# DLR-RM/AugmentedAutoencoder

Measured on AMD Instinct MI355X. Metric: crops/sec (encode+codebook-NN), 128x128x3 vs 92232x128 codebook, 1/8 GPU, higher is better.
Workload: dtype f32; 1 GPU; configs[1]: single object per GPU, batch=256 uint8 128x128x3 crops, HIP 4-conv encoder -> 128-d + cosine-NN vs 92232x128 fp32 codebook, top-1; batch_per_gpu=256, codebook_rows=92232, latent=128, parallelism=single GPU

## Files before the change

augmentedautoencoder_amd/csrc/kernels/conv_winograd_f32.h:

```cpp
#pragma once
#include <type_traits>

#include "multi_launch.h"

namespace aae {

struct ConvWinoArgs {
    const float* x;
    const float* U;
    const float* bias;
    const float* bn_scale;
    const float* bn_shift;
    float* out;
    int B, H, W, Cin, Cout, Ho, Wo;
    int eh, ew;
    int mode;
    int relu;
    int blocks_x, blocks_y;
    int regions;
    int xcd_cols;
#ifdef AAE_WINO_STAMPS
    long long* stamps;
#endif
};
#ifdef AAE_WINO_STAMPS
constexpr int kWinoStampSlots = 48;
#define AAE_WINO_STAMP(a, slot) do { if ((threadIdx.x & 63) == 0) (a).stamps[((size_t)blockIdx.x * 8 + (threadIdx.x >> 6)) * aae::kWinoStampSlots + (slot)] = aae::clock_ticks(); } while (0)
#else
#define AAE_WINO_STAMP(a, slot) do {} while (0)
#endif
inline unsigned wino_grid_blocks(int regions, int nbn, int xcd_cols) {
    if (xcd_cols <= 0) return (unsigned)regions * (unsigned)nbn;
    const int region_groups = 8 / (nbn / xcd_cols);
    return 8u * (unsigned)xcd_cols * (unsigned)((regions + region_groups - 1) / region_groups);
}
inline bool wino_xcd_cols_valid(int nbn, int xcd_cols) {
    return xcd_cols >= 1 && nbn % xcd_cols == 0 && (nbn / xcd_cols) <= 8 && 8 % (nbn / xcd_cols) == 0;
}

template <int GEOM>
struct WinoGeom;
template <>
struct WinoGeom<0> {
    static constexpr int kImages = 1, kRows = 18, kCols = 18, kRowPitch = 12, kParityPitch = 220, kImagePitch = 2 * 220;
};
template <>
struct WinoGeom<1> {
    static constexpr int kImages = 4, kRows = 10, kCols = 10, kRowPitch = 6, kParityPitch = 60, kImagePitch = 128;
};
template <int GEOM>
constexpr int wino_plane_units() { return WinoGeom<GEOM>::kImages * WinoGeom<GEOM>::kImagePitch + 1; }
template <int GEOM>
constexpr int wino_stage_units() { return 8 * wino_plane_units<GEOM>(); }
template <int GEOM>
constexpr int wino_smem_bytes() { return 2 * wino_stage_units<GEOM>() * 16; }

struct ConvWinoLayerArgs {
    ConvWinoArgs c;
    const float* U4[4];
};
struct ConvWinoObject {
    const float* x;
    float* out;
    const float* U4[4];
    const float* bias;
    const float* bn_scale;
    const float* bn_shift;
    int B, pad_;
};
struct ConvWinoMultiArgs {
    ConvWinoArgs c;
    MultiRange range;
    ConvWinoObject obj[kMultiMax];
};
template <int GEOM>
constexpr int wino_layer_stage_bytes() { return 2 * 4 * wino_plane_units<GEOM>() * 16; }
template <int GEOM>
constexpr int wino_layer_smem_bytes() { return wino_layer_stage_bytes<GEOM>() + 4 * 64 * 64 * 4; }


#ifndef AAE_WINO_DECLARATIONS_ONLY

#if defined(__HIP_DEVICE_COMPILE__)
__device__ __forceinline__ f32x2 wino_pk_add(f32x2 a, f32x2 b) {
    f32x2 r;
    asm("v_pk_add_f32 %0, %1, %2" : "=v"(r) : "v"(a), "v"(b));
    return r;
}
__device__ __forceinline__ f32x2 wino_pk_sub(f32x2 a, f32x2 b) {
    f32x2 r;
    asm("v_pk_add_f32 %0, %1, %2 neg_lo:[0,1] neg_hi:[0,1]" : "=v"(r) : "v"(a), "v"(b));
    return r;
}
#else
__host__ __device__ inline f32x2 wino_pk_add(f32x2 a, f32x2 b) { return a + b; }
__host__ __device__ inline f32x2 wino_pk_sub(f32x2 a, f32x2 b) { return a - b; }
#endif
#if defined(__HIP_DEVICE_COMPILE__)
__device__ __forceinline__ f32x4 wino_fma4(float s, f32x4 a, f32x4 b) {
    const f32x2 ss = {s, s};
    f32x2 lo, hi;
    asm("v_pk_fma_f32 %0, %1, %2, %3" : "=v"(lo) : "v"(ss), "v"(a.lo), "v"(b.lo));
    asm("v_pk_fma_f32 %0, %1, %2, %3" : "=v"(hi) : "v"(ss), "v"(a.hi), "v"(b.hi));
    return f32x4{lo.x, lo.y, hi.x, hi.y};
}
#else
__host__ __device__ inline f32x4 wino_fma4(float s, f32x4 a, f32x4 b) {
    f32x4 r;
    for (int e = 0; e < 4; ++e) r[e] = fmaf(s, a[e], b[e]);
    return r;
}
#endif
__device__ __forceinline__ f32x4 wino_add4(f32x4 a, f32x4 b) {
    const f32x2 lo = wino_pk_add(a.lo, b.lo), hi = wino_pk_add(a.hi, b.hi);
    return f32x4{lo.x, lo.y, hi.x, hi.y};
}
__device__ __forceinline__ f32x4 wino_sub4(f32x4 a, f32x4 b) {
    const f32x2 lo = wino_pk_sub(a.lo, b.lo), hi = wino_pk_sub(a.hi, b.hi);
    return f32x4{lo.x, lo.y, hi.x, hi.y};
}

struct WinoBlock {
    int nb, region, img0, wy0, wx0;
    bool live;
};
__device__ __forceinline__ void wino_block_index(int block, int nbn, int regions, int xcd_cols, WinoBlock& w) {
    if (xcd_cols > 0) {
        const int col_groups = nbn / xcd_cols, region_groups = 8 / col_groups, chunk = (regions + region_groups - 1) / region_groups;
        const int xcd = block & 7, within = block >> 3, k = within / xcd_cols;
        w.nb = (xcd % col_groups) * xcd_cols + within % xcd_cols;
        w.region = (xcd / col_groups) * chunk + k;
        w.live = k < chunk && w.region < regions;
    } else {
        w.nb = block % nbn;
        w.region = block / nbn;
        w.live = w.region < regions;
    }
}
template <int GEOM>
__device__ __forceinline__ void wino_block_geometry(int local, int blocks_x, int blocks_y, WinoBlock& w) {
    if (GEOM == 0) {
        int rest = local;
        const int bx = rest % blocks_x;
        rest /= blocks_x;
        const int by = rest % blocks_y;
        w.img0 = rest / blocks_y;
        w.wy0 = 16 * by - 1;
        w.wx0 = 16 * bx - 1;
    } else {
        w.img0 = 4 * local;
        w.wy0 = w.wx0 = -1;
    }
}
template <int GEOM>
__device__ __forceinline__ WinoBlock wino_block(int block, int nbn, int blocks_x, int blocks_y, int regions, int xcd_cols) {
    WinoBlock w;
    wino_block_index(block, nbn, regions, xcd_cols, w);
    wino_block_geometry<GEOM>(w.region, blocks_x, blocks_y, w);
    return w;
}
template <int GEOM>
__device__ __forceinline__ void wino_tile(int mh, int t, int& ti, int& ty, int& tx) {
    if (GEOM == 0) { ti = 0; ty = 4 * mh + (t >> 3); tx = t & 7; }
    else { ti = 2 * mh + (t >> 4); ty = (t >> 2) & 3; tx = t & 3; }
}



template <int GEOM, int STAGE_CH, int NT>
struct WinoFillPlan {
    static constexpr int kQuads = STAGE_CH / 4, kParts = STAGE_CH / 16;
    static constexpr int kStageQuads = WinoGeom<GEOM>::kImages * WinoGeom<GEOM>::kRows * WinoGeom<GEOM>::kCols * kQuads;
    static constexpr int kPer = ((kStageQuads + NT - 1) / NT + kParts - 1) / kParts;
    uint32_t goff[kParts * kPer];
    int lslot[kParts * kPer];
};
constexpr uint32_t kWinoOutside = 0x80000000u;
template <int GEOM, int STAGE_CH, int NT>
__device__ __forceinline__ void wino_fill_plan(const ConvWinoArgs& a, const WinoBlock& wb, WinoFillPlan<GEOM, STAGE_CH, NT>& f) {
    using G = WinoGeom<GEOM>;
    using F = WinoFillPlan<GEOM, STAGE_CH, NT>;
    constexpr int kPlane = wino_plane_units<GEOM>();
    const int cq_per_pixel = a.Cin / 4;
#pragma unroll
    for (int i = 0; i < F::kParts * F::kPer; ++i) {
        const int idx = (int)threadIdx.x + NT * i;
        f.goff[i] = kWinoOutside;
        f.lslot[i] = -1;
        if (idx < F::kStageQuads) {
            const int pixel = idx / F::kQuads, cq = idx - pixel * F::kQuads;
            const int wi = pixel / (G::kRows * G::kCols), rem = pixel - wi * (G::kRows * G::kCols);
            const int wy = rem / G::kCols, wx = rem - wy * G::kCols;
            const int uu = wb.wy0 + wy, vv = wb.wx0 + wx, b = wb.img0 + wi;
            if (uu >= 0 && uu < a.Ho && vv >= 0 && vv < a.Wo && b < a.B)
                f.goff[i] = (uint32_t)(((((size_t)b * a.H + 2 * uu) * a.W + 2 * vv) * cq_per_pixel + cq) * 16);
            f.lslot[i] = cq * kPlane + wi * G::kImagePitch + (wx & 1) * G::kParityPitch + wy * G::kRowPitch + (wx >> 1);
        }
    }
}

template <int TA, int TB, bool SWAP, int GEOM, int STAGE_CH, bool ACCUMULATE, bool WIDE, int CHAIN = 0, int NTA = 3, int NTB = 3>
__device__ __forceinline__ void wino_phase_body(const ConvWinoArgs& a, const float* U, int eh, int ew, const WinoBlock& wb, f32x4* lds, float* xch_all,
                                                const WinoFillPlan<GEOM, STAGE_CH, WIDE ? 256 : 512>& fill, int& buf0, f32x4 (&uin)[8],
                                                const float* Un, int neh, int new_, f32x4 (&uout)[8]) {
    using G = WinoGeom<GEOM>;
    using F = WinoFillPlan<GEOM, STAGE_CH, WIDE ? 256 : 512>;
    constexpr int PB = TB + 1;
    constexpr int kQuads = STAGE_CH / 4, kGroups = STAGE_CH / 8;
    constexpr int kPlane = wino_plane_units<GEOM>(), kStage = kQuads * kPlane;
    constexpr int kParity = G::kParityPitch;
    constexpr int kParts = F::kParts, kPer = F::kPer;
    constexpr int NH = WIDE ? 2 : 1;
    constexpr int kOffA = TA == 2 ? 1 : 0, kOffB = TB == 2 ? 1 : 0;
    static_assert(CHAIN == 0 || !WIDE, "the chained form passes one wave's weight fragments between the components");
    const int tid = threadIdx.x, lane = tid & 63, wave = tid >> 6;
    const int mh = wave & 1, nh = WIDE ? 0 : (wave >> 1) & 1, ph = WIDE ? wave >> 1 : wave >> 2, m = lane & 31, h = lane >> 5;
    int li, lty, ltx;
    wino_tile<GEOM>(mh, m, li, lty, ltx);
    const int n32 = wb.nb * 2 + nh, KG = a.Cin / 8, nst = a.Cin / STAGE_CH;
    constexpr int NP = (TA + 1) * PB;
    constexpr int kPhaseNo = TA == 3 && TB == 3 ? 0 : (TA == 3 && !SWAP ? 1 : (TA == 3 ? 2 : 3));
    (void)kPhaseNo;
    AAE_WINO_STAMP(a, 4 * kPhaseNo + 0);
    const buffer_rsrc xrs = make_buffer(a.x, (uint32_t)((size_t)a.B * a.H * a.W * a.Cin * 4));
    const buffer_rsrc urs = make_buffer(U, (uint32_t)((size_t)NP * a.Cin * a.Cout * 4));
    const uint32_t ulane = (uint32_t)(((size_t)n32 * KG * NP + (size_t)ph * 2 * PB) * 64 + h * 32 + m) * 16u;
    const bool two_rows = TA == 3 || ph == 0;
    const uint32_t parity_off = (uint32_t)(((size_t)eh * a.W + ew) * a.Cin * 4);
    const uint32_t next_parity_off = (uint32_t)(((size_t)neh * a.W + new_) * a.Cin * 4);

    f32x16 acc[NH][2 * PB];
#pragma unroll
    for (int n2 = 0; n2 < NH; ++n2)
#pragma unroll
        for (int p = 0; p < 2 * PB; ++p)
#pragma unroll
            for (int r = 0; r < 16; ++r) acc[n2][p][r] = 0.f;

    f32x4 stg[kPer];
    auto stage_load = [&](uint32_t soff, int part) {
#pragma unroll
        for (int i = 0; i < kPer; ++i) stg[i] = buffer_load4_s(xrs, fill.goff[part * kPer + i], soff);
    };
    auto stage_store = [&](int buf, int part) {
#pragma unroll
        for (int i = 0; i < kPer; ++i)
            if (fill.lslot[part * kPer + i] >= 0) lds[buf * kStage + fill.lslot[part * kPer + i]] = stg[i];
    };
    auto fA = [](int pos) { return SWAP ? (pos & 1) * kParity + (pos >> 1) : pos * G::kRowPitch; };
    auto fB = [](int pos) { return SWAP ? pos * G::kRowPitch : (pos & 1) * kParity + (pos >> 1); };
    const int lane_base = li * G::kImagePitch + 2 * lty * G::kRowPitch + ltx;
    const int posA0 = (TA == 3 ? (ph == 0 ? 0 : 2) : (ph == 0 ? 0 : 1)) + kOffA;
    const int posA1 = (ph == 0 ? 1 : 3) + kOffA;
    const int posA2 = (TA == 3 ? (ph == 0 ? 2 : 1) : (ph == 0 ? 1 : 2)) + kOffA;
    const int offA0 = fA(posA0), offA1 = fA(posA1), offA2 = fA(posA2);
    const float sg = ph == 0 ? 1.f : -1.f;

    const uint32_t half_stride = (uint32_t)KG * NP * 1024u;
    f32x4 u[NH][2 * PB];
    if (CHAIN & 1) {
#pragma unroll
        for (int p = 0; p < 2 * PB; ++p) u[0][p] = uin[p];
    } else {
#pragma unroll
        for (int n2 = 0; n2 < NH; ++n2)
#pragma unroll
            for (int p = 0; p < 2 * PB; ++p)
                u[n2][p] = buffer_load4_s(urs, ulane + (p % PB) * 1024u, (two_rows ? (p / PB) * PB * 1024u : (p / PB) * (NP * 1024u)) + n2 * half_stride);
#pragma unroll
        for (int part = 0; part < kParts; ++part) {
            stage_load(parity_off, part);
            stage_store(buf0, part);
        }
        __syncthreads();
    }
    AAE_WINO_STAMP(a, 4 * kPhaseNo + 1);

    auto read_unit = [&](const f32x4* plane, int i, f32x4 (&raw)[2 * PB]) {
#pragma unroll
        for (int s2 = 0; s2 < PB; ++s2) {
            const int ob = fB(s2 + kOffB);
            if (i == 0) raw[s2] = plane[offA0 + ob];
            else if (TA == 3) raw[s2] = plane[offA1 + ob];
            raw[PB + s2] = plane[offA2 + ob];
        }
    };
    auto step_a = [&](int i, const f32x4 (&raw)[2 * PB], f32x4 (&w)[PB]) {
#pragma unroll
        for (int s2 = 0; s2 < PB; ++s2) {
            if (i == 0) w[s2] = wino_sub4(raw[s2], raw[PB + s2]);
            else if (TA == 3) w[s2] = wino_fma4(sg, raw[s2], raw[PB + s2]);
            else w[s2] = raw[PB + s2];
        }
    };
    auto step_b = [&](f32x4 (&w)[PB]) {
        if (TB == 3) {
            const f32x4 e0 = w[0], e1 = w[1], e2 = w[2], e3 = w[PB - 1];
            w[0] = wino_sub4(e0, e2);
            w[1] = wino_add4(e1, e2);
            w[2] = wino_sub4(e2, e1);
            w[PB - 1] = wino_sub4(e1, e3);
        } else {
            const f32x4 e0 = w[0], e1 = w[1], e2 = w[2];
            w[0] = wino_sub4(e0, e1);
            w[2] = wino_sub4(e1, e2);
        }
    };
    auto run = [&](auto rows_tag) {
        constexpr int ROWS = decltype(rows_tag)::value, NU = kGroups * ROWS, kPartUnits = NU / kParts;
        static_assert(NU % 2 == 0 && NU % kParts == 0, "units per stage");
        constexpr int kStoreBack = (kParts == 1 && NU >= 4) ? 2 : 1;
        const bool early = ph == 1 && NU >= 4 && kParts == 1;
        f32x4 raw[2 * PB], v[PB];
        read_unit(lds + buf0 * kStage + h * kPlane + lane_base, 0, raw);
        for (int st = 0; st < nst; ++st) {
            const int buf = (buf0 + st) & 1;
            const bool more = st + 1 < nst;
            const bool filling = more || (CHAIN & 2);
            const uint32_t fill_off = more ? parity_off + (uint32_t)(st + 1) * kQuads * 16 : next_parity_off;
#ifdef AAE_WINO_STAMPS
            if (kPhaseNo == 0 && st < 8) AAE_WINO_STAMP(a, 20 + st);
#endif
            const f32x4* stage = lds + buf * kStage + h * kPlane + lane_base;
            const f32x4* next_stage = lds + (buf ^ 1) * kStage + h * kPlane + lane_base;
#pragma unroll
            for (int t = 0; t < NU; ++t) {
                const int i = t % ROWS, slot = t & 1;
#ifdef AAE_WINO_STAMPS
                if (kPhaseNo == 0 && (st == 2 || st == 3) && t < 4) AAE_WINO_STAMP(a, 28 + 6 * (st - 2) + t);
#endif
                step_a(i, raw, v);
                step_b(v);
                if ((st > 0 || t > 0) && (more || t + 1 < NU)) {
                    const int tn = (t + 1) % NU, gn = (st + (t + 1) / NU) * kGroups + tn / ROWS;
                    const uint32_t un = (uint32_t)gn * (NP * 1024u) + (tn % ROWS) * PB * 1024u;
#pragma unroll
                    for (int n2 = 0; n2 < NH; ++n2)
#pragma unroll
                        for (int j = 0; j < PB; ++j) u[n2][(slot ^ 1) * PB + j] = buffer_load4_s(urs, ulane + j * 1024u, un + n2 * half_stride);
                }
                if (filling && t % kPartUnits == 0) stage_load(fill_off, t / kPartUnits);
                if (filling && t % kPartUnits == kPartUnits - kStoreBack) stage_store(buf ^ 1, t / kPartUnits);
                if (t + 1 < NU) read_unit(stage + 2 * ((t + 1) / ROWS) * kPlane, (t + 1) % ROWS, raw);
                if (filling && (t == NU - 1 ? !early : (t == NU - 2 && early))) {
#ifdef AAE_WINO_STAMPS
                    if (kPhaseNo == 0 && (st == 2 || st == 3)) AAE_WINO_STAMP(a, 28 + 6 * (st - 2) + 4);
#endif
                    __syncthreads();
#ifdef AAE_WINO_STAMPS
                    if (kPhaseNo == 0 && (st == 2 || st == 3)) AAE_WINO_STAMP(a, 28 + 6 * (st - 2) + 5);
#endif
                }
                if (t == NU - 1 && more) read_unit(next_stage, 0, raw);
                sched_fence();
#pragma unroll
                for (int q = 0; q < 4; ++q)
#pragma unroll
                    for (int j = 0; j < PB; ++j)
#pragma unroll
                        for (int n2 = 0; n2 < NH; ++n2)
                            acc[n2][(ROWS == 2 ? i * PB : 0) + j] = mfma_32x32x2(v[j][q], u[n2][slot * PB + j][q], acc[n2][(ROWS == 2 ? i * PB : 0) + j]);
                sched_fence();
            }
        }
    };
    if (TA == 3 || ph == 0) run(std::integral_constant<int, 2>());
    else run(std::integral_constant<int, 1>());
    if (STAGE_CH == 32 && !(CHAIN & 2)) __syncthreads();
    AAE_WINO_STAMP(a, 4 * kPhaseNo + 2);
    if (CHAIN & 2) {
        constexpr int NPB = NTB + 1, NNP = (NTA + 1) * NPB;
        const buffer_rsrc nrs = make_buffer(Un, (uint32_t)((size_t)NNP * a.Cin * a.Cout * 4));
        const uint32_t nlane = (uint32_t)(((size_t)n32 * KG * NNP + (size_t)ph * 2 * NPB) * 64 + h * 32 + m) * 16u;
        const bool next_two_rows = NTA == 3 || ph == 0;
#pragma unroll
        for (int p = 0; p < 2 * NPB; ++p)
            uout[p] = buffer_load4_s(nrs, nlane + (p % NPB) * 1024u, next_two_rows ? (p / NPB) * NPB * 1024u : (p / NPB) * (NNP * 1024u));
    }
    buf0 = (buf0 + nst) & 1;

    auto partial = [&](int n2, int r, float (&y)[4]) {
        float q0[PB], q1[PB];
#pragma unroll
        for (int j = 0; j < PB; ++j) {
            const float mA = acc[n2][j][r], mB = acc[n2][PB + j][r];
            if (ph == 0) { q0[j] = mA + mB; q1[j] = mB; }
            else if (TA == 3) { q0[j] = mA; q1[j] = -mA - mB; }
            else { q0[j] = 0.f; q1[j] = -mA; }
        }
        float t[4];
        if (TB == 3) {
            t[0] = q0[0] + q0[1] + q0[2];
            t[1] = q0[1] - q0[2] - q0[3];
            t[2] = q1[0] + q1[1] + q1[2];
            t[3] = q1[1] - q1[2] - q1[3];
        } else {
            t[0] = q0[0] + q0[1];
            t[1] = q0[1] - q0[2];
            t[2] = q1[0] + q1[1];
            t[3] = q1[1] - q1[2];
        }
        y[0] = t[0];
        y[1] = SWAP ? t[2] : t[1];
        y[2] = SWAP ? t[1] : t[2];
        y[3] = t[3];
    };
    f32x4 yv[NH][16];
#pragma unroll
    for (int n2 = 0; n2 < NH; ++n2)
#pragma unroll
        for (int r = 0; r < 16; ++r) {
            float y[4];
            partial(n2, r, y);
            yv[n2][r] = f32x4{y[0], y[1], y[2], y[3]};
        }
#pragma unroll
    for (int round = 0; round < 2; ++round) {
#pragma unroll
        for (int n2 = 0; n2 < NH; ++n2) {
            f32x4* xq = reinterpret_cast<f32x4*>(xch_all) + (size_t)(mh + 2 * (nh + n2)) * 16 * 64 + lane;
            if (ACCUMULATE || round == 1) {
                f32x4 old[8];
#pragma unroll
                for (int e = 0; e < 8; ++e) old[e] = ph == round ? xq[(2 * e) * 64] : xq[(2 * e + 1) * 64];
#pragma unroll
                for (int e = 0; e < 8; ++e) {
                    if (ph == round) xq[(2 * e) * 64] = old[e] + yv[n2][2 * e];
                    else xq[(2 * e + 1) * 64] = old[e] + yv[n2][2 * e + 1];
                }
            } else {
#pragma unroll
                for (int e = 0; e < 8; ++e) {
                    if (ph == round) xq[(2 * e) * 64] = yv[n2][2 * e];
                    else xq[(2 * e + 1) * 64] = yv[n2][2 * e + 1];
                }
            }
        }
        __syncthreads();
    }
    AAE_WINO_STAMP(a, 4 * kPhaseNo + 3);
}

template <int GEOM, int NT>
__device__ __forceinline__ void wino_store_block(const ConvWinoArgs& a, int mode, const WinoBlock& wb, const float* xall) {
    const int tid = threadIdx.x;
    const int n4 = wb.nb * 64 + (tid & 15) * 4;
    f32x4 bs = {0.f, 0.f, 0.f, 0.f}, sc = {1.f, 1.f, 1.f, 1.f}, sh = {0.f, 0.f, 0.f, 0.f};
    if (mode >= 2) {
        bs = *reinterpret_cast<const f32x4*>(a.bias + n4);
        if (a.bn_scale) {
            sc = *reinterpret_cast<const f32x4*>(a.bn_scale + n4);
            sh = *reinterpret_cast<const f32x4*>(a.bn_shift + n4);
        }
    }
#pragma unroll
    for (int round = 0; round < 1024 / NT; ++round) {
        const int idx = tid + NT * round, cq = idx & 15, t = idx >> 4;
        const int tmh = t >> 5, mt = t & 31, tnh = cq >> 3;
        const int r = (mt & 3) + 4 * (mt >> 3), hh = (mt >> 2) & 1;
        const f32x4* src = reinterpret_cast<const f32x4*>(xall) + (size_t)(tmh + 2 * tnh) * 16 * 64 + r * 64 + 32 * hh + (cq & 7) * 4;
        const f32x4 c0 = src[0], c1 = src[1], c2 = src[2], c3 = src[3];
        int ti, ty, tx;
        wino_tile<GEOM>(tmh, mt, ti, ty, tx);
        const int b = wb.img0 + ti;
        if (b >= a.B) continue;
        const int oy = (GEOM == 0 ? wb.wy0 + 1 : 0) + 2 * ty, ox = (GEOM == 0 ? wb.wx0 + 1 : 0) + 2 * tx;
        float* o = a.out + (((size_t)b * a.Ho + oy) * a.Wo + ox) * a.Cout + wb.nb * 64 + cq * 4;
        float* optr[4] = {o, o + a.Cout, o + (size_t)a.Wo * a.Cout, o + (size_t)a.Wo * a.Cout + a.Cout};
        f32x4 val[4];
#pragma unroll
        for (int k = 0; k < 4; ++k) val[k] = f32x4{c0[k], c1[k], c2[k], c3[k]};
        if (mode == 1 || mode == 2) {
#pragma unroll
            for (int k = 0; k < 4; ++k) val[k] += *reinterpret_cast<const f32x4*>(optr[k]);
        }
        if (mode >= 2) {
#pragma unroll
            for (int k = 0; k < 4; ++k) {
                val[k] += bs;
                if (a.relu) {
#pragma unroll
                    for (int e = 0; e < 4; ++e) val[k][e] = fmaxf(val[k][e], 0.f);
                }
                if (a.bn_scale) val[k] = val[k] * sc + sh;
            }
        }
#pragma unroll
        for (int k = 0; k < 4; ++k) *reinterpret_cast<f32x4*>(optr[k]) = val[k];
    }
}

#ifdef AAE_EXPERIMENTS
template <int TA, int TB, bool SWAP, int GEOM>
__global__ __launch_bounds__(512) void conv_wino_phase_kernel(ConvWinoArgs a) {
    AAE_DYN_SMEM(smem_raw);
    const WinoBlock wb = wino_block<GEOM>(blockIdx.x, a.Cout / 64, a.blocks_x, a.blocks_y, a.regions, a.xcd_cols);
    if (!wb.live) return;
    WinoFillPlan<GEOM, 32, 512> fill;
    wino_fill_plan(a, wb, fill);
    int buf0 = 0;
    f32x4 unused[8];
    wino_phase_body<TA, TB, SWAP, GEOM, 32, false, false>(a, a.U, a.eh, a.ew, wb, reinterpret_cast<f32x4*>(smem_raw), reinterpret_cast<float*>(smem_raw), fill, buf0, unused,
                                                          nullptr, 0, 0, unused);
    wino_store_block<GEOM, 512>(a, a.mode, wb, reinterpret_cast<const float*>(smem_raw));
}
#endif

template <int GEOM, bool WIDE>
__device__ __forceinline__ void wino_layer_block(const ConvWinoArgs& a, const float* const (&U4)[4], const WinoBlock& wb, unsigned char* smem_raw) {
    f32x4* lds = reinterpret_cast<f32x4*>(smem_raw);
    float* xch = reinterpret_cast<float*>(smem_raw + wino_layer_stage_bytes<GEOM>());
    WinoFillPlan<GEOM, 16, WIDE ? 256 : 512> fill;
    wino_fill_plan(a, wb, fill);
    int buf0 = 0;
    f32x4 ua[8], ub[8];
    if (WIDE) {
        wino_phase_body<3, 3, false, GEOM, 16, false, WIDE>(a, U4[3], 1, 1, wb, lds, xch, fill, buf0, ua, nullptr, 0, 0, ub);
        wino_phase_body<3, 2, false, GEOM, 16, true, WIDE>(a, U4[2], 1, 0, wb, lds, xch, fill, buf0, ua, nullptr, 0, 0, ub);
        wino_phase_body<3, 2, true, GEOM, 16, true, WIDE>(a, U4[1], 0, 1, wb, lds, xch, fill, buf0, ua, nullptr, 0, 0, ub);
        wino_phase_body<2, 2, false, GEOM, 16, true, WIDE>(a, U4[0], 0, 0, wb, lds, xch, fill, buf0, ua, nullptr, 0, 0, ub);
    } else {
        constexpr bool W = WIDE;
        wino_phase_body<3, 3, false, GEOM, 16, false, W, W ? 0 : 2, 3, 2>(a, U4[3], 1, 1, wb, lds, xch, fill, buf0, ua, U4[2], 1, 0, ub);
        wino_phase_body<3, 2, false, GEOM, 16, true, W, W ? 0 : 3, 3, 2>(a, U4[2], 1, 0, wb, lds, xch, fill, buf0, ub, U4[1], 0, 1, ua);
        wino_phase_body<3, 2, true, GEOM, 16, true, W, W ? 0 : 3, 2, 2>(a, U4[1], 0, 1, wb, lds, xch, fill, buf0, ua, U4[0], 0, 0, ub);
        wino_phase_body<2, 2, false, GEOM, 16, true, W, W ? 0 : 1>(a, U4[0], 0, 0, wb, lds, xch, fill, buf0, ub, nullptr, 0, 0, ua);
    }
    wino_store_block<GEOM, WIDE ? 256 : 512>(a, 3, wb, xch);
}

template <int GEOM, bool WIDE>
__global__ __launch_bounds__(WIDE ? 256 : 512) void conv_wino_layer_kernel(ConvWinoLayerArgs p) {
    AAE_DYN_SMEM(smem_raw);
    const ConvWinoArgs& a = p.c;
    const WinoBlock wb = wino_block<GEOM>(blockIdx.x, a.Cout / 64, a.blocks_x, a.blocks_y, a.regions, a.xcd_cols);
    if (!wb.live) return;
    wino_layer_block<GEOM, WIDE>(a, p.U4, wb, smem_raw);
#ifdef AAE_WINO_STAMPS
    asm volatile("s_waitcnt vmcnt(0)" ::: "memory");
    AAE_WINO_STAMP(a, 16);
    if (threadIdx.x == 0) a.stamps[((size_t)blockIdx.x * 8) * kWinoStampSlots + 17] = (long long)(__builtin_amdgcn_s_getreg(20 | (0 << 6) | (3 << 11)) & 15);
#endif
}

template <int GEOM>
__global__ __launch_bounds__(512) void conv_wino_layer_multi_kernel(ConvWinoMultiArgs p) {
    AAE_DYN_SMEM(smem_raw);
    WinoBlock wb;
    wino_block_index(blockIdx.x, p.c.Cout / 64, p.c.regions, p.c.xcd_cols, wb);
    if (!wb.live) return;
    const int o = multi_find(p.range, wb.region);
    wino_block_geometry<GEOM>(wb.region - p.range.first[o], p.c.blocks_x, p.c.blocks_y, wb);
    ConvWinoArgs a = p.c;
    const ConvWinoObject& ob = p.obj[o];
    a.x = ob.x; a.out = ob.out; a.bias = ob.bias; a.bn_scale = ob.bn_scale; a.bn_shift = ob.bn_shift; a.B = ob.B;
    const float* U4[4] = {ob.U4[0], ob.U4[1], ob.U4[2], ob.U4[3]};
    wino_layer_block<GEOM, false>(a, U4, wb, smem_raw);
}

#endif

}
```

Measured before the change: 54460 crops/s.

## Specialize Winograd output drain per phase and drop trailing barrier when chained

The output-transform drain is split into two compile-time specializations on the wave's phase, so branches on ph and its select-based LDS addressing become static. It uses inline asm adds, and an accumulator fence with s_nops to keep MFMA results ordered before the drain. Redundant LDS reads in read_unit for later rows are dropped, and the final __syncthreads after the second exchange round is skipped when the chained next phase has at least two stages. Together these cut VALU/LDS overhead and a barrier, but risk correctness if the skipped barrier was needed, plus code size and register pressure from two drain copies.

```diff
diff --git a/augmentedautoencoder_amd/csrc/kernels/conv_winograd_f32.h b/augmentedautoencoder_amd/csrc/kernels/conv_winograd_f32.h
--- a/augmentedautoencoder_amd/csrc/kernels/conv_winograd_f32.h
+++ b/augmentedautoencoder_amd/csrc/kernels/conv_winograd_f32.h
@@ -24,7 +24,7 @@
 #endif
 };
 #ifdef AAE_WINO_STAMPS
-constexpr int kWinoStampSlots = 48;
+constexpr int kWinoStampSlots = 64;
 #define AAE_WINO_STAMP(a, slot) do { if ((threadIdx.x & 63) == 0) (a).stamps[((size_t)blockIdx.x * 8 + (threadIdx.x >> 6)) * aae::kWinoStampSlots + (slot)] = aae::clock_ticks(); } while (0)
 #else
 #define AAE_WINO_STAMP(a, slot) do {} while (0)
@@ -118,6 +118,39 @@
 __device__ __forceinline__ f32x4 wino_sub4(f32x4 a, f32x4 b) {
     const f32x2 lo = wino_pk_sub(a.lo, b.lo), hi = wino_pk_sub(a.hi, b.hi);
     return f32x4{lo.x, lo.y, hi.x, hi.y};
+}
+#if defined(__HIP_DEVICE_COMPILE__)
+__device__ __forceinline__ float wino_add1(float a, float b) {
+    float r;
+    asm("v_add_f32 %0, %1, %2" : "=v"(r) : "v"(a), "v"(b));
+    return r;
+}
+__device__ __forceinline__ float wino_sub1(float a, float b) {
+    float r;
+    asm("v_sub_f32 %0, %1, %2" : "=v"(r) : "v"(a), "v"(b));
+    return r;
+}
+__device__ __forceinline__ float wino_nadd1(float a, float b) {
+    float r;
+    asm("v_sub_f32 %0, -%1, %2" : "=v"(r) : "v"(a), "v"(b));
+    return r;
+}
+#else
+__host__ __device__ inline float wino_add1(float a, float b) { return a + b; }
+__host__ __device__ inline float wino_sub1(float a, float b) { return a - b; }
+__host__ __device__ inline float wino_nadd1(float a, float b) { return -a - b; }
+#endif
+template <int N>
+__device__ __forceinline__ void wino_acc_fence(f32x16 (&c)[N]) {
+#if defined(__HIP_DEVICE_COMPILE__)
+    static_assert(N == 6 || N == 8, "2 PB accumulator tiles");
+    if constexpr (N == 8)
+        asm volatile("s_nop 15\n\ts_nop 3" : "+v"(c[0]), "+v"(c[1]), "+v"(c[2]), "+v"(c[3]), "+v"(c[4]), "+v"(c[5]), "+v"(c[6]), "+v"(c[7]));
+    else
+        asm volatile("s_nop 15\n\ts_nop 3" : "+v"(c[0]), "+v"(c[1]), "+v"(c[2]), "+v"(c[3]), "+v"(c[4]), "+v"(c[5]));
+#else
+    (void)c;
+#endif
 }
 
 struct WinoBlock {
@@ -213,7 +246,7 @@
     constexpr int NH = WIDE ? 2 : 1;
     constexpr int kOffA = TA == 2 ? 1 : 0, kOffB = TB == 2 ? 1 : 0;
     static_assert(CHAIN == 0 || !WIDE, "the chained form passes one wave's weight fragments between the components");
-    const int tid = threadIdx.x, lane = tid & 63, wave = tid >> 6;
+    const int tid = threadIdx.x, lane = tid & 63, wave = wave_uniform(tid >> 6);
     const int mh = wave & 1, nh = WIDE ? 0 : (wave >> 1) & 1, ph = WIDE ? wave >> 1 : wave >> 2, m = lane & 31, h = lane >> 5;
     int li, lty, ltx;
     wino_tile<GEOM>(mh, m, li, lty, ltx);
@@ -282,7 +315,7 @@
             const int ob = fB(s2 + kOffB);
             if (i == 0) raw[s2] = plane[offA0 + ob];
             else if (TA == 3) raw[s2] = plane[offA1 + ob];
-            raw[PB + s2] = plane[offA2 + ob];
+            if (i == 0) raw[PB + s2] = plane[offA2 + ob];
         }
     };
     auto step_a = [&](int i, const f32x4 (&raw)[2 * PB], f32x4 (&w)[PB]) {
@@ -378,66 +411,79 @@
             uout[p] = buffer_load4_s(nrs, nlane + (p % NPB) * 1024u, next_two_rows ? (p / NPB) * NPB * 1024u : (p / NPB) * (NNP * 1024u));
     }
     buf0 = (buf0 + nst) & 1;
-
-    auto partial = [&](int n2, int r, float (&y)[4]) {
-        float q0[PB], q1[PB];
-#pragma unroll
-        for (int j = 0; j < PB; ++j) {
-            const float mA = acc[n2][j][r], mB = acc[n2][PB + j][r];
-            if (ph == 0) { q0[j] = mA + mB; q1[j] = mB; }
-            else if (TA == 3) { q0[j] = mA; q1[j] = -mA - mB; }
-            else { q0[j] = 0.f; q1[j] = -mA; }
-        }
-        float t[4];
-        if (TB == 3) {
-            t[0] = q0[0] + q0[1] + q0[2];
-            t[1] = q0[1] - q0[2] - q0[3];
-            t[2] = q1[0] + q1[1] + q1[2];
-            t[3] = q1[1] - q1[2] - q1[3];
-        } else {
-            t[0] = q0[0] + q0[1];
-            t[1] = q0[1] - q0[2];
-            t[2] = q1[0] + q1[1];
-            t[3] = q1[1] - q1[2];
-        }
-        y[0] = t[0];
-        y[1] = SWAP ? t[2] : t[1];
-        y[2] = SWAP ? t[1] : t[2];
-        y[3] = t[3];
-    };
-    f32x4 yv[NH][16];
-#pragma unroll
-    for (int n2 = 0; n2 < NH; ++n2)
-#pragma unroll
-        for (int r = 0; r < 16; ++r) {
-            float y[4];
-            partial(n2, r, y);
-            yv[n2][r] = f32x4{y[0], y[1], y[2], y[3]};
-        }
-#pragma unroll
-    for (int round = 0; round < 2; ++round) {
-#pragma unroll
-        for (int n2 = 0; n2 < NH; ++n2) {
-            f32x4* xq = reinterpret_cast<f32x4*>(xch_all) + (size_t)(mh + 2 * (nh + n2)) * 16 * 64 + lane;
-            if (ACCUMULATE || round == 1) {
-                f32x4 old[8];
-#pragma unroll
-                for (int e = 0; e < 8; ++e) old[e] = ph == round ? xq[(2 * e) * 64] : xq[(2 * e + 1) * 64];
-#pragma unroll
-                for (int e = 0; e < 8; ++e) {
-                    if (ph == round) xq[(2 * e) * 64] = old[e] + yv[n2][2 * e];
-                    else xq[(2 * e + 1) * 64] = old[e] + yv[n2][2 * e + 1];
-                }
+#pragma unroll
+    for (int n2 = 0; n2 < NH; ++n2) wino_acc_fence(acc[n2]);
+
+    auto drain = [&](auto ph_tag) {
+        constexpr int PH = decltype(ph_tag)::value;
+        auto partial = [&](int n2, int r, float (&y)[4]) {
+            constexpr bool kNoQ0 = PH == 1 && TA == 2;
+            float q0[PB], q1[PB];
+#pragma unroll
+            for (int j = 0; j < PB; ++j) {
+                const float mA = acc[n2][j][r], mB = acc[n2][PB + j][r];
+                if (PH == 0) { q0[j] = wino_add1(mA, mB); q1[j] = mB; }
+                else if (TA == 3) { q0[j] = mA; q1[j] = wino_nadd1(mA, mB); }
+                else { q0[j] = 0.f; q1[j] = -mA; }
+            }
+            float t[4];
+            if (TB == 3) {
+                t[0] = kNoQ0 ? 0.f : wino_add1(wino_add1(q0[0], q0[1]), q0[2]);
+                t[1] = kNoQ0 ? 0.f : wino_sub1(wino_sub1(q0[1], q0[2]), q0[3]);
+                t[2] = wino_add1(wino_add1(q1[0], q1[1]), q1[2]);
+                t[3] = wino_sub1(wino_sub1(q1[1], q1[2]), q1[3]);
             } else {
-#pragma unroll
-                for (int e = 0; e < 8; ++e) {
-                    if (ph == round) xq[(2 * e) * 64] = yv[n2][2 * e];
-                    else xq[(2 * e + 1) * 64] = yv[n2][2 * e + 1];
+                t[0] = kNoQ0 ? 0.f : wino_add1(q0[0], q0[1]);
+                t[1] = kNoQ0 ? 0.f : wino_sub1(q0[1], q0[2]);
+                t[2] = wino_add1(q1[0], q1[1]);
+                t[3] = wino_sub1(q1[1], q1[2]);
+            }
+            y[0] = t[0];
+            y[1] = SWAP ? t[2] : t[1];
+            y[2] = SWAP ? t[1] : t[2];
+            y[3] = t[3];
+        };
+        f32x4 yv[NH][16];
+#pragma unroll
+        for (int n2 = 0; n2 < NH; ++n2)
+#pragma unroll
+            for (int r = 0; r < 16; ++r) {
+                float y[4];
+                partial(n2, r, y);
+                yv[n2][r] = f32x4{y[0], y[1], y[2], y[3]};
+            }
+#ifdef AAE_WINO_STAMPS
+        AAE_WINO_STAMP(a, 48 + 4 * kPhaseNo + 0);
+#endif
+#pragma unroll
+        for (int round = 0; round < 2; ++round) {
+            const int par = PH == round ? 0 : 1;
+#pragma unroll
+            for (int n2 = 0; n2 < NH; ++n2) {
+                f32x4* xq = reinterpret_cast<f32x4*>(xch_all) + (size_t)(mh + 2 * (nh + n2)) * 16 * 64 + lane;
+                if (ACCUMULATE || round == 1) {
+                    f32x4 old[8];
+#pragma unroll
+                    for (int e = 0; e < 8; ++e) old[e] = xq[(2 * e + par) * 64];
+#pragma unroll
+                    for (int e = 0; e < 8; ++e) xq[(2 * e + par) * 64] = old[e] + yv[n2][2 * e + par];
+                } else {
+#pragma unroll
+                    for (int e = 0; e < 8; ++e) xq[(2 * e + par) * 64] = yv[n2][2 * e + par];
                 }
             }
-        }
-        __syncthreads();
-    }
+#ifdef AAE_WINO_STAMPS
+            asm volatile("s_waitcnt lgkmcnt(0)" ::: "memory");
+            AAE_WINO_STAMP(a, 48 + 4 * kPhaseNo + 1 + 2 * round);
+#endif
+            if (round == 0 || !(CHAIN & 2) || nst < 2) __syncthreads();
+#ifdef AAE_WINO_STAMPS
+            if (round == 0) AAE_WINO_STAMP(a, 48 + 4 * kPhaseNo + 2);
+#endif
+        }
+    };
+    if (ph == 0) drain(std::integral_constant<int, 0>());
+    else drain(std::integral_constant<int, 1>());
     AAE_WINO_STAMP(a, 4 * kPhaseNo + 3);
 }
 
```

Measured after the change: 55720 crops/s (median of 6 runs). 2.3% higher.
